# buggyyang/CDC_compression

Measured on AMD Instinct MI355X. Metric: decoded images/sec at 256x256, 500-step x-param, higher is better.
Workload: dtype f32 (f16x2 split products)

## Files before the change

### cdc_compression_amd/csrc/cdc_internal.h

```cpp
#pragma once
#include <stdio.h>
#include <string.h>
#include <stdlib.h>
#include <hip/hip_runtime.h>
#include <map>
#include <mutex>
#include <utility>
#include <stdint.h>

#include <string>
#include <vector>

#include "conv_args.h"

extern "C" char **environ;

namespace cdc {

typedef void (*conv_kernel_fn)(const ConvArgs);
conv_kernel_fn conv_lookup_a(int MB, int NPW, int lnmode);
conv_kernel_fn conv_lookup_b(int MB, int NPW, int lnmode);
conv_kernel_fn conv_lookup_c(int MB, int NPW, int lnmode);
conv_kernel_fn conv_lookup_split(int MB, int NPW);
conv_kernel_fn conv_lookup_split2(int MB, int NPW, int lnmode, int xu = 1);
conv_kernel_fn conv_lookup_split2h(int MB, int NPW, int lnmode, int xu = 1);
conv_kernel_fn conv_lookup_split2hu(int MB, int NPW);

struct ConvShape {
    int Cin, Cout, KH, KW, stride;
    int C0 = 0;
    int Win = 0;
    int nz = 1, pad_x[4] = {0, 0, 0, 0};
    bool allow_split = false;
    int arith = 0;
    bool per_image_w = false;
    int Ho, Wo;
    int B;
    bool need_all_cout;
    int lnmode;
    int max_ksplit = 1;
};
bool conv_make_plan(const ConvShape &s, ConvPlan *plan);
hipError_t conv_launch(ConvArgs a, const ConvPlan &plan, int B, int nz, hipStream_t st);

struct PfShape {
    int Cin, Cout, C0 = 0, KH, KW, nz = 1, Ho, Wo, B;
    bool need_all_cout = false;
    int stride = 1;
    int uf = 0;
    int cop = 0;
    int tz = 1;
};
struct PfPlan {
    int MB, NPW, WM, WP, ring, tiles_x, tiles_y, groups; size_t lds_bytes; int lin = 0;
    int x16 = 0;
    int pf3_epv = 0, pf3_G = 0, pf3_iters = 0;
};
bool pf_make_plan(const PfShape &s, PfPlan *plan);
hipError_t pf_launch(PfArgs a, const PfPlan &plan, int B, int nz, hipStream_t st);
bool pf3_make_plan(const PfArgs &a, int B, int nz, PfPlan *plan);
hipError_t pf3_launch(PfArgs a, const PfPlan &plan, int B, hipStream_t st);
int device_cus();
struct WsPlan { int W, NPB, stride, waves, tiles, groups; size_t lds_bytes; };
struct WsArgs;
bool ws_make_plan(int Cin, int C0, int Cout, int H, int W, int B, int stride, WsPlan *plan);
hipError_t ws_launch(WsArgs a, const WsPlan &plan, hipStream_t st);
struct Ws1Plan { int NPB, waves, tiles, groups; size_t lds_bytes; };
struct Ws1Args;
bool ws1_make_plan(int Cin, int C0, int Cout, int HW, int B, bool per_image_w, Ws1Plan *plan);
hipError_t ws1_launch(Ws1Args a, const Ws1Plan &plan, hipStream_t st);
bool pw_make_plan(const PfShape &s, PfPlan *plan);
hipError_t pw_launch(PfArgs a, const PfPlan &plan, int B, hipStream_t st);
hipError_t pf_pack_launch(const float *src, long long src_bs, void *dst, long long dst_bs, int C, int H, int W, int B,
                          hipStream_t st);
hipError_t c4_pack_launch(const float *src, long long src_bs, float *dst, int C, long long HW, int B, hipStream_t st);
hipError_t pf_unpack_launch(const void *src, long long src_bs, float *dst, long long dst_bs, int C, int H, int W, int B, hipStream_t st);

inline const char *dev_env(const char *name) {
    static const bool on = [] {
        const char *e = ::getenv("CDC_DEV");
        if (e && atoi(e) != 0) return true;
        static const char *const user_level[] = {"CDC_DEV=", "CDC_ARITH=", "CDC_NO_RANGE_GUARD=", "CDC_GRAPH=", "CDC_DEBUG_PLAN=", "CDC_PROF_OPS=",
                                                 "CDC_BENCH_", "CDC_TEST_OBS=", "CDC_SYNC_EACH_OP=", "CDC_HIP_LIB=", "CDC_NO_COMBINE_FUSE="};
        for (char **v = environ; v && *v; ++v) {
            if (strncmp(*v, "CDC_", 4)) continue;
            bool user = false;
            for (const char *u : user_level) user = user || !strncmp(*v, u, strlen(u));
            if (!user) {
                fprintf(stderr, "cdc_hip: %.*s is set but ignored: development switches need CDC_DEV=1\n", (int)strcspn(*v, "="), *v);
                break;
            }
        }
        return false;
    }();
    return on ? ::getenv(name) : nullptr;
}

inline hipError_t ensure_dynamic_lds(const void *fn, size_t bytes) {
    if (bytes <= 64 * 1024) return hipSuccess;
    static std::mutex mu;
    static std::map<std::pair<int, const void *>, size_t> done;
    int dev = 0;
    (void)hipGetDevice(&dev);
    std::lock_guard<std::mutex> lk(mu);
    size_t &have = done[{dev, fn}];
    if (have >= bytes) return hipSuccess;
    hipError_t e = hipFuncSetAttribute(fn, hipFuncAttributeMaxDynamicSharedMemorySize, (int)bytes);
    if (e == hipSuccess) have = bytes;
    return e;
}

__host__ __device__ inline int ceil_div(int a, int b) { return (a + b - 1) / b; }
__host__ __device__ inline int round_up(int a, int b) { return ceil_div(a, b) * b; }

struct LnArgs {
    const float *in;
    float *out;
    int C, HW;
    const float *g, *b;
    float eps;
    int relu;
    const float *shift;
    int shift_bs;
    const float *resid;
    float *stat_mean, *stat_rstd;
    int nparts;
    long long part_stride;
    int *fault;
    int img_major;
};
hipError_t ln_launch(const LnArgs &a, int B, hipStream_t st);

struct TembLayer {
    const float *w, *bias;
    int cout;
    int out_off;
};
struct TembArgs {
// ... 151 lines not shown
```

### cdc_compression_amd/csrc/cdc_planner.hip

```cpp
#include "cdc_state.h"

namespace cdcapi {

constexpr int kKsTarget = 1024;

struct Builder {
    cdc_handle *h;
    int B;
    std::vector<void *> *pool;
    int rc = CDC_OK;
    int planB = 0;
    int pb() const { return planB > 0 ? planB : B; }
    std::vector<Op> *cur = nullptr;

    void emit(Op op) {
        op.id = (int)h->op_ms.size();
        h->op_ms.push_back(0); h->op_n.push_back(0); h->op_flops.push_back(op.flops);
        const bool hoisted = cur == &h->pre_ops;
        char buf[160];
        std::visit([&](const auto &payload) { op_label(payload, buf, sizeof buf, hoisted); }, op.p);
        if (hoisted && !strstr(buf, " HOIST") && strlen(buf) + 7 < sizeof buf) strcat(buf, " HOIST");
        h->op_label.push_back(buf);
        (cur ? cur : &h->ops)->push_back(op);
    }
// ... 249 lines not shown
        if (t0->H != H || t0->W != W || (t1 && (t1->H != H || t1->W != W))) return false;
        if (s1 ? (t0->C != C0 || t0->C + t1->C != w.Cin) : t0->C != w.Cin) return false;
        PfPlan plan;
        if (!pf_make_plan(ps, &plan)) return false;
        const int Ho = ps.Ho, Wo = ps.Wo;
        PfConvOp op;
        op.plan = plan; op.nz = w.nz;
        PfArgs &a = op.a;
        memset(&a, 0, sizeof a);
        a.src0 = t0->p; a.src0_bs = t0->bs();
        if (t1) { a.src1 = t1->p; a.src1_bs = t1->bs(); }
        a.C0 = s1 ? C0 : w.Cin; a.Cin = w.Cin; a.H = H; a.W = W;
        a.w = w.wsh; a.w_zs = w.wsp_zs / 8;
        a.KH = w.KH; a.KW = w.KW; a.nz = w.nz; a.stride = w.stride; a.tz = ps.tz;
        a.nchunk = w.Cin / 16; a.COP = w.COP; a.Cout = w.Cout;
        a.acc_scale = w.wscale_inv;
        out_geometry(a, w, Ho, Wo);
        a.out = out; a.out_bs = out_bs;
        if (o.emit_pf && bind_out_pf(a, w, out, out_bs, Ho, Wo) && o.no_f32) a.out = nullptr;
        epilogue(a, w, o);
        if (o.resid1) {
            if (!o.resid || o.resid_c0 <= 0 || o.resid_c0 >= w.Cout || (o.resid_c0 % 64) || (o.resid_c0 % (plan.MB * 32))) return false;
            a.resid1 = o.resid1; a.resid1_bs = o.resid1_bs; a.resid_c0 = o.resid_c0;
        }
        if (PfTwin *tr = o.resid ? twin(o.resid) : nullptr)
            if (tr->only) {
                if (!tr->valid || tr->C != w.Cout || tr->H != Ho || tr->W != Wo || w.transposed || w.stride != 1 ||
                    o.resid_bs != (long long)w.Cout * Ho * Wo || o.resid_cs != (long long)Ho * Wo) {
                    if (!ensure_f32(o.resid, o.resid_bs)) {
                        if (!rc) rc = fail(h, CDC_ERR_UNSUPPORTED, "planes-only residual of a shape the plane-operand kernels do not read");
                        return true;
                    }
                } else {
                    a.resid = nullptr;
                    a.resid_pf = tr->p; a.rpf_bs = tr->bs(); a.rpf_ps = tr->ps(); a.rpf_ys = Wo + 2; a.rpf_zoff = (Wo + 2) + 1;
                }
            }
        if (planB == 0) pf3_make_plan(a, B, w.nz, &op.plan);
        if (debug_plan())
            fprintf(stderr, "[plan] conv %dx%d %d->%d out %dx%d on conv_pf%s_kernel (epv %d, %d workgroups x %d tiles per group)\n", w.KH, w.KW, w.Cin, w.Cout,
                    Ho, Wo, op.plan.pf3_epv ? "3" : "", op.plan.pf3_epv, op.plan.pf3_G, op.plan.pf3_iters);
        const double px = (double)B * Ho * Wo * w.nz;
        return finish(prof, op, 2.0 * px * w.Cout * w.Cin * w.KH * w.KW, 4.0 * ((double)B * w.Cin * H * W + px * w.Cout), a.out == nullptr);
    }

    bool try_pf_uf(const ConvW &w, const float *s0, long long bs0, int H, int W, float *out, long long out_bs, const ConvOpts &o,
                   bool need_all, int prof) {
        PfShape ps;
        if (!pf_on() || o.uf_c != 3 || o.uf_pad != 3 || !pf_uf_form(w, H, W, need_all, &ps)) return false;
        if (o.pre_mean || o.w_bs || o.wsp_bs || o.max_ksplit > 1 || o.resid || o.res3_w || o.stat_mean) return false;
        PfPlan plan;
        if (!pf_make_plan(ps, &plan)) return false;
        PfConvOp op;
        op.plan = plan; op.nz = 1;
        PfArgs &a = op.a;
        memset(&a, 0, sizeof a);
        a.x0 = s0; a.x0_bs = bs0;
        a.C0 = a.Cin = 32; a.H = H; a.W = W;
        a.w = w.wsh; a.w_zs = w.wsp_zs / 8;
        a.KH = 7; a.KW = 1; a.nz = 1;
        a.nchunk = 2; a.COP = w.COP; a.Cout = w.Cout;
        a.acc_scale = w.wscale_inv;
        out_geometry(a, w, H, W);
        a.out = out; a.out_bs = out_bs;
        if (o.emit_pf && bind_out_pf(a, w, out, out_bs, H, W) && o.no_f32) a.out = nullptr;
        const float *c4 = o.pre_add && cur != &h->pre_ops ? pre_add_c4(o.pre_add, w.Cout, H, W, out_bs) : nullptr;
        epilogue(a, w, o);
        if (c4) { a.pre_add = c4; a.pre_c4 = 1; }
        const double px = (double)B * H * W;
        return finish(prof, op, 2.0 * px * w.Cout * w.Cin * 7, 4.0 * ((double)B * 3 * H * W + px * w.Cout), a.out == nullptr);
    }

    bool try_pw(const ConvW &w, const float *s0, int C0, long long bs0, const float *s1, long long bs1, int H, int W,
                float *out, long long out_bs, const ConvOpts &o, bool need_all, int prof) {
        PfShape ps;
        if (h->arith != 1 || dev_env("CDC_NO_PW") || !pw_form(w, s1 ? C0 : 0, H, W, &ps)) return false;
        if (need_all || o.ln_g || o.stat_mean || o.res3_w || o.pf_only) return false;
        if (o.pre_mean && o.pre_mode != 2) return false;
        if (o.w_bs && !o.wsp_bs) return false;
        PfPlan plan;
        if (!pw_make_plan(ps, &plan)) return false;
        if (plan.lin && (o.shift || o.wsp_bs || (long long)w.Cout * H * W != out_bs)) return false;
        if (debug_plan())
            fprintf(stderr, "[plan] conv1x1 PW Cin=%4d Cout=%4d out=%3dx%-3d %s%s| MB=%d NPW=%d WM=%d WP=%d groups=%d R=%d wgs=%d lds=%zu\n", w.Cin, w.Cout,
                    H, W, o.pre_mean ? "pre2 " : "", o.wsp_bs ? "per-image " : "", plan.MB, plan.NPW, plan.WM, plan.WP, plan.groups, plan.ring,
                    plan.tiles_x * plan.tiles_y * B * plan.groups, plan.lds_bytes);
        PwConvOp op;
        op.plan = plan;
        PfArgs &a = op.a;
        memset(&a, 0, sizeof a);
        a.x0 = s0; a.x0_bs = bs0; a.x1 = s1; a.x1_bs = bs1;
        a.C0 = s1 ? C0 : w.Cin; a.Cin = w.Cin; a.H = H; a.W = W;
        a.pre_mean = o.pre_mean; a.pre_rstd = o.pre_mean ? o.pre_rstd : nullptr;
        a.w = w.wsh; a.w_bs = o.wsp_bs / 8;
        a.KH = 1; a.KW = 1; a.nz = 1;
        a.nchunk = w.Cin / 16; a.COP = w.COP; a.Cout = w.Cout;
        a.acc_scale = w.wscale_inv;
        out_geometry(a, w, H, W);
        a.out = out; a.out_bs = out_bs;
        if (o.emit_pf && !plan.lin && (w.Cout % 32) == 0 && bind_out_pf(a, w, out, out_bs, H, W) && o.no_f32) a.out = nullptr;
        epilogue(a, w, o);
        const double px = (double)B * H * W;
        return finish(prof, op, 2.0 * px * w.Cout * w.Cin, 4.0 * ((double)B * w.Cin * H * W + px * w.Cout), a.out == nullptr);
    }

    bool ws_would_plan(const ConvW &w, int C0, bool two_src, int H, int W, WsPlan *plan) {
        if (h->arith != 1 || !w.wsh || planB > 0 || w.KH != 3 || w.KW != 3 || (w.stride != 1 && w.stride != 2) || w.transposed || w.nz != 1) return false;
        if (w.py() != 1 || w.px() != 1) return false;
        if (w.COP != w.Cout || w.Cin_pad != w.Cin) return false;
        if (w.stride == 2 && ((H & 1) || (W & 1) || two_src)) return false;
        return ws_make_plan(w.Cin, two_src ? C0 : w.Cin, w.Cout, H / w.stride, W / w.stride, pb(), w.stride, plan);
    }
    bool try_ws(const ConvW &w, const float *s0, int C0, long long bs0, const float *s1, long long bs1, int H, int W, float *raw,
                long long raw_bs, int prof, const float *pre_add = nullptr) {
        WsConvOp op;
        if (rc || !ws_would_plan(w, C0, s1 != nullptr, H, W, &op.plan)) return false;
        if (!ensure_f32(s0, bs0) || (s1 && !ensure_f32(s1, bs1))) return false;
        const int Ho = H / w.stride, Wo = W / w.stride;
        if (raw_bs != (long long)w.Cout * Ho * Wo) return false;
        WsArgs &a = op.a;
        memset(&a, 0, sizeof a);
        a.x0 = s0; a.x0_bs = bs0; a.x1 = s1; a.x1_bs = bs1;
        a.C0 = s1 ? C0 : w.Cin; a.Cin = w.Cin; a.H = Ho; a.B = B;
        a.w = w.wsh; a.nchunk = w.Cin / 16; a.COP = w.COP; a.Cout = w.Cout; a.acc_scale = w.wscale_inv;
        a.bias = pre_add ? nullptr : w.bias;
        a.pre_add = pre_add;
        a.out = raw; a.out_bs = raw_bs;
        a.fault = fault_flag();
        if (debug_plan())
            fprintf(stderr, "[plan] conv 3x3 s%d %d->%d out %dx%d on conv_ws_kernel: %d tiles of %d pixels x %d groups, %d waves, %zu bytes of LDS\n", w.stride, w.Cin, w.Cout, Ho, Wo,
                    op.plan.tiles, op.plan.NPB * 32, op.plan.groups, op.plan.waves, op.plan.lds_bytes);
        const double px = (double)B * Ho * Wo;
        return finish(prof, op, 2.0 * px * w.Cout * w.Cin * 9, 4.0 * ((double)B * H * W * w.Cin + px * w.Cout), false);
    }

    bool try_ws1(const ConvW &w, const float *s0, int C0, long long bs0, const float *s1, long long bs1, int H, int W, float *out, long long out_bs,
                 const ConvOpts &o, bool need_all, int prof) {
        PfShape ps;
        if (rc || h->arith != 1 || planB > 0 || !pw_form(w, 0, H, W, &ps)) return false;
        if (need_all || o.ln_g || o.stat_mean || o.res3_w || o.pf_only || (o.pre_add && o.resid) || o.relu || o.resid1 || o.uf_c) return false;
        if (o.pre_mean && o.pre_mode != 2) return false;
        if (o.w_bs && !o.wsp_bs) return false;
        if (w.COP != w.Cout || w.Cin_pad != w.Cin || out_bs != (long long)w.Cout * H * W) return false;
        if (o.resid && (o.resid_cs != (long long)H * W)) return false;
        const long long blocks = (long long)pb() * (H * W / 32);
        const long long max_blocks = dev_env("CDC_WS1_MAX_BLOCKS") ? atoll(dev_env("CDC_WS1_MAX_BLOCKS")) : 128;
        const int max_groups_wide = dev_env("CDC_WS1_MAX_GROUPS") ? atoi(dev_env("CDC_WS1_MAX_GROUPS")) : 0;
        const bool wide_ok = blocks <= max_blocks || (max_groups_wide > 0 && blocks <= 256 && w.Cout / 32 <= max_groups_wide);
        if (!wide_ok && !(o.wsp_bs && W < 32)) return false;
        Ws1ConvOp op;
        op.H = H;
        if (!ws1_make_plan(w.Cin, s1 ? C0 : w.Cin, w.Cout, H * W, pb(), o.wsp_bs != 0, &op.plan)) return false;
        if (!ensure_f32(s0, bs0) || (s1 && !ensure_f32(s1, bs1)) || (o.resid && !ensure_f32(o.resid, o.resid_bs))) return false;
        Ws1Args &a = op.a;
        memset(&a, 0, sizeof a);
        a.x0 = s0; a.x0_bs = bs0; a.x1 = s1; a.x1_bs = bs1;
        a.C0 = s1 ? C0 : w.Cin; a.Cin = w.Cin; a.HW = H * W; a.B = B;
        a.pre_mean = o.pre_mean; a.pre_rstd = o.pre_mean ? o.pre_rstd : nullptr;
        a.w = w.wsh; a.w_bs = o.wsp_bs / 8;
        a.nchunk = w.Cin / 16; a.COP = w.COP; a.Cout = w.Cout; a.acc_scale = w.wscale_inv;
        a.bias = o.no_bias ? nullptr : w.bias;
        a.shift = o.shift; a.shift_bs = shift_stride(o);
        a.resid = o.resid; a.resid_bs = o.resid_bs;
        if (o.pre_add) { a.resid = o.pre_add; a.resid_bs = out_bs; a.resid_is_pre = 1; }
        a.out = out; a.out_bs = out_bs;
        a.fault = fault_flag();
        if (debug_plan())
            fprintf(stderr, "[plan] conv 1x1 %d->%d out %dx%d on conv_ws1_kernel: %d tiles of %d pixels x %d groups, %d waves%s%s\n", w.Cin, w.Cout, H, W,
                    op.plan.tiles, op.plan.NPB * 32, op.plan.groups, op.plan.waves, o.pre_mean ? ", folded PreNorm" : "", o.wsp_bs ? ", per-image weights" : "");
// ... 1072 lines not shown
```

### cdc_compression_amd/csrc/conv_args.h

```cpp
#pragma once
#include <stdint.h>

namespace cdc {

constexpr int kWaveSize = 64;
constexpr int kXS = 20;

struct ConvArgs {
    const float *src0, *src1;
    long long src0_bs, src1_bs;
    int uf_c, uf_pad;
    unsigned uf_magic;
    int C0, Cin;
    int H, W;
    const float *ln_mean, *ln_rstd;
    const float *ln_g, *ln_b;
    const float *wp;
    long long w_bs, w_zs;
    const unsigned short *wsp;
    long long wsp_zs;
    long long wsp_bs;
    float acc_scale;
    int tg;
    int ipw, B;
// ... 3 lines not shown
    float *out;
    long long out_bs, out_cs;
    int out_ys, out_xs, out_zoff[4];
    int Ho, Wo;
    int lognbw;
    int tiles_x, tiles_y;
    int PH, PW;
    int xvec, xshift[4];
    unsigned magic_hw, magic_w;
    const float *bias;
    const float *pre_add;
    const float *ep_g, *ep_b;
    float eps;
    int relu;
    float relu_slope;
    const float *shift;
    int shift_bs;
    const float *resid;
    long long resid_bs, resid_cs;
    const float *res3_w, *res3_x;
    long long res3_bs;
    float *stat_mean, *stat_rstd;
    int ksplit, nzz;
    int xcd_remap;
    int zfold;
    long long out_ks;
    void *out_pf;
    long long pf_bs, pf_ps;
    int pf_ys, pf_xs, pf_zoff[4];
    int pf_only;
    int *fault;
#ifdef CDC_TIMELINE
    unsigned long long *tl;
#endif
};

struct PfArgs {
    const void *src0, *src1;
    long long src0_bs, src1_bs;
    int C0, Cin;
    int H, W;
    const void *w;
    long long w_zs;
    int KH, KW, nz;
    int stride;
    int tz;
    int pad_y[4], pad_x[4];
    int nchunk, COP, Cout;
    float acc_scale;
    int ring;
    int n_iter;
    float *out;
    long long out_bs, out_cs;
    int out_ys, out_xs, out_zoff[4];
    void *out_pf;
    long long pf_bs, pf_ps;
    int pf_ys, pf_xs, pf_zoff[4];
    int Ho, Wo;
    int lognbw, tiles_x, tiles_y, B;
    int xcd_remap;
    const float *bias, *pre_add, *ep_g, *ep_b;
    int pre_c4;
    float eps;
    int relu;
    float relu_slope;
    const float *shift;
    int shift_bs;
    const float *resid;
    long long resid_bs, resid_cs;
    const float *resid1;
    long long resid1_bs;
    int resid_c0;
    const void *resid_pf;
    long long rpf_bs, rpf_ps;
    int rpf_ys, rpf_zoff;
    float *stat_mean, *stat_rstd;
    const float *res3_w, *res3_x;
    long long res3_bs;
    const float *x0, *x1;
    long long x0_bs, x1_bs;
    const float *pre_mean, *pre_rstd;
    long long w_bs;
    int lin;
    int dbg;
    int *fault;
#ifdef CDC_TIMELINE
    unsigned long long *tl;
#endif
};

constexpr int kPfXS = 12;

struct ConvPlan {
    int MB, NPW, WN;
    int groups;
    int KC, nchunk;
    int lognbw, tiles_x, tiles_y, PH, PW;
    int xvec, xshift[4];
    size_t lds_bytes;
    int lnmode;
    int tg;
    int ipw;
    int ksplit = 1;
    int xu = 1;
    int arith = 0;
    int split;
};

}
```

### cdc_compression_amd/csrc/conv_inst_w.hip

```cpp
#include <algorithm>
#include <map>
#include <string>
#include <vector>
#include <stdlib.h>

#include "cdc_internal.h"
#include "conv_pw_kernel.h"

namespace cdc {

typedef void (*pw_kernel_fn)(const PfArgs);
static pw_kernel_fn pw_lookup(int MB, int NPW, int WM, int WP, bool x16 = false) {
    if (x16) {
        if (MB == 2 && NPW == 2 && WM == 1 && WP == 4) return conv_pw_kernel<2, 2, 1, 4, true>;
        if (MB == 2 && NPW == 2 && WM == 2 && WP == 2) return conv_pw_kernel<2, 2, 2, 2, true>;
        if (MB == 2 && NPW == 2 && WM == 4 && WP == 2) return conv_pw_kernel<2, 2, 4, 2, true>;
        if (MB == 3 && NPW == 1 && WM == 2 && WP == 4) return conv_pw_kernel<3, 1, 2, 4, true>;
        return nullptr;
    }
    if (MB == 2 && NPW == 2 && WM == 1 && WP == 4) return conv_pw_kernel<2, 2, 1, 4>;
    if (MB == 2 && NPW == 2 && WM == 2 && WP == 2) return conv_pw_kernel<2, 2, 2, 2>;
    if (MB == 2 && NPW == 2 && WM == 4 && WP == 2) return conv_pw_kernel<2, 2, 4, 2>;
    if (MB == 3 && NPW == 1 && WM == 2 && WP == 4) return conv_pw_kernel<3, 1, 2, 4>;
    return nullptr;
}
struct PwCand { int MB, NPW, WM, WP; };
static const PwCand kPwCands[] = {
    {2, 2, 4, 2},
    {3, 1, 2, 4},
    {2, 2, 2, 2},
    {2, 2, 1, 4},
};

bool pw_make_plan(const PfShape &s, PfPlan *p) {
    if (s.KH != 1 || s.KW != 1 || s.nz != 1) return false;
    if (s.Cout % 32 || s.Cin % 16 || (s.C0 % 16) || s.Cin < 32) return false;
    const bool lin = s.Wo < 32;
    if (lin && ((s.Ho * s.Wo) % 32)) return false;
    const double min_waves = dev_env("CDC_PW_MIN_WAVES") ? atof(dev_env("CDC_PW_MIN_WAVES")) : 512.0;
    const bool x16 = (lin || ((s.Wo & 3) == 0 && s.Wo >= 4)) && !dev_env("CDC_NO_PW_X16");
    double best = -1;
    for (const PwCand &c : kPwCands) {
        const int COPT = c.WM * c.MB * 32, NW = c.WM * c.WP;
        if (s.Cout % COPT) continue;
        if (s.need_all_cout && COPT != s.Cout) continue;
        const int ring = pw_ring(c.MB, c.NPW, c.WM, c.WP, x16);
        if (ring < 5 || s.Cin / 16 < 2) continue;
        const int TH = c.WP * c.NPW;
        const int groups = s.Cout / COPT;
        const long long nb = (long long)s.B * (s.Ho * s.Wo / 32);
        const double wgs = lin ? (double)((nb + TH - 1) / TH) * groups
                               : (double)((s.Wo + 31) / 32) * ((s.Ho + TH - 1) / TH) * s.B * groups;
        if (wgs * NW < min_waves) continue;
        const double fill = std::min(1.0, wgs * NW / 2048.0);
        const double score = fill / (1.0 + 0.25 * (groups - 1)) * (c.MB * c.NPW >= 4 ? 1.0 : 0.8);
        if (score > best) {
            best = score;
            p->MB = c.MB; p->NPW = c.NPW; p->WM = c.WM; p->WP = c.WP;
            p->ring = ring;
            p->lin = lin ? 1 : 0;
            p->tiles_x = lin ? (int)((nb + TH - 1) / TH) : (s.Wo + 31) / 32;
            p->tiles_y = lin ? 1 : (s.Ho + TH - 1) / TH;
            p->groups = groups;
            p->lds_bytes = (size_t)ring * pf_rows(c.MB, c.NPW) * COPT * 16 + pw_x_bytes(c.NPW, c.WM, c.WP, x16);
            p->x16 = x16 ? 1 : 0;
        }
    }
    return best >= 0;
}

hipError_t pw_launch(PfArgs a, const PfPlan &p, int B, hipStream_t st) {
    pw_kernel_fn fn = pw_lookup(p.MB, p.NPW, p.WM, p.WP, p.x16 != 0);
    if (!fn) return hipErrorInvalidValue;
    a.lognbw = 5;
    a.tiles_x = p.tiles_x; a.tiles_y = p.tiles_y; a.B = B; a.ring = p.ring;
    if (hipError_t e = ensure_dynamic_lds((const void *)fn, p.lds_bytes); e != hipSuccess) return e;
    a.lin = p.lin;
    if (const char *e = dev_env("CDC_PW_DBG")) a.dbg = atoi(e); else
    a.dbg = dev_env("CDC_PW_COUNTED_WAIT") ? 1024 : 0;
    dim3 grid((unsigned)(p.lin ? p.tiles_x : p.tiles_x * p.tiles_y * B), (unsigned)p.groups, 1);
    a.xcd_remap = (grid.x % 8 == 0 && grid.x >= 64) ? 1 : 0;
#ifdef CDC_TIMELINE
    static unsigned long long *tl_dev = nullptr;
    static std::map<std::string, int> seen;
    const size_t tl_wgs = (size_t)grid.x * grid.y;
    char key[96];
    snprintf(key, sizeof key, "pw 1x1 %d->%d out %dx%d", a.Cin, a.Cout, a.Ho, a.Wo);
    a.tl = nullptr;
    if (tl_wgs <= (1u << 18) && seen[key]++ < 2) {
        if (!tl_dev) hipMalloc(&tl_dev, sizeof(unsigned long long) * 16 * (1u << 18));
        hipMemsetAsync(tl_dev, 0, sizeof(unsigned long long) * 16 * tl_wgs, st);
        a.tl = tl_dev;
    }
#endif
    hipLaunchKernelGGL(fn, grid, dim3(64 * p.WM * p.WP), p.lds_bytes, st, a);
#ifdef CDC_TIMELINE
    if (a.tl) {
        hipStreamSynchronize(st);
        std::vector<unsigned long long> h(16 * tl_wgs);
        hipMemcpy(h.data(), tl_dev, h.size() * 8, hipMemcpyDeviceToHost);
        double cat[7] = {0}, life = 0;
        for (size_t w = 0; w < tl_wgs; ++w) {
            const unsigned long long *r = &h[w * 16];
            for (int c = 0; c < 7; ++c) cat[c] += (double)r[c];
            life += (double)(r[8] - r[7]);
        }
        static const char *names[7] = {"setup", "prologue issue", "prologue wait", "main loop", "epilogue parameters", "-", "epilogue blocks"};
        fprintf(stderr, "[pf timeline] conv %s: %zu workgroups x %d threads, lds %zu; mean workgroup life %.0f; per workgroup (wave 0):", key, tl_wgs, 64 * p.WM * p.WP, p.lds_bytes,
                life / tl_wgs);
        for (int c = 0; c < 7; ++c) fprintf(stderr, "  %s %.0f", names[c], cat[c] / tl_wgs);
        fprintf(stderr, "\n");
    }
#endif
    return hipGetLastError();
}

}
```

### cdc_compression_amd/csrc/conv_pw_kernel.h

```cpp
#pragma once
#include "conv_pf_kernel.h"

namespace cdc {

constexpr int kPwPD = 2;
constexpr int kPwX16N = 2 * 256 + 32;
__host__ __device__ constexpr size_t pw_x_bytes(int NPW, int WM, int WP, bool X16 = false) {
    return (size_t)WM * WP * kPwPD * NPW * (X16 ? kPwX16N * 4 : 8 * 256);
}
__host__ __device__ constexpr int pw_ring(int MB, int NPW, int WM, int WP, bool X16 = false) {
    const size_t budget = (WM * WP == 8 ? 150 * 1024 : 78 * 1024) - pw_x_bytes(NPW, WM, WP, X16);
    const size_t wst = (size_t)pf_rows(MB, NPW) * WM * MB * 32 * 16;
    const int r = (int)(budget / wst);
    return r > 6 ? 6 : r;
}

__device__ __forceinline__ void dma4(unsigned voff, const void *sbase, unsigned lds_byte) {
    asm volatile("s_mov_b32 m0, %2\n\ts_nop 0\n\tglobal_load_lds_dword %0, %1" ::"v"(voff), "s"(sbase), "s"(lds_byte)
                 : "memory");
}

template <int MB, int NPW, int WM, int WP, bool X16 = false>
__global__ void __launch_bounds__(64 * WM * WP, WM * WP == 8 ? 1 : 2) conv_pw_kernel(const PfArgs P) {
    constexpr int NW = WM * WP, NT = 64 * NW, COPT = WM * MB * 32;
    static_assert(COPT % 64 == 0, "a weight DMA instruction (64 units) must stay inside one (plane, k-half) row");
    constexpr bool ACC2 = pf_acc2(MB, NPW);
    constexpr int NPL = ACC2 ? 2 : 3, ROWS = 2 * NPL;
    constexpr int WI = ROWS * COPT / 64;
    constexpr int NWW = (WI + NW - 1) / NW;
    constexpr int WST = ROWS * COPT;
    constexpr int R = pw_ring(MB, NPW, WM, WP, X16);
    static_assert(R >= 5, "no room for the weight ring");
    constexpr int TH = WP * NPW;
    constexpr int PD = kPwPD;
    extern __shared__ __attribute__((aligned(16))) uint4 smem_u[];
#ifdef CDC_TIMELINE
    unsigned long long tl_acc[7] = {0, 0, 0, 0, 0, 0, 0}, tl_last = __builtin_readcyclecounter();
    const unsigned long long tl_start = tl_last;
#endif
    const int tid = threadIdx.x, lane = tid & 63;
    const int wave = __builtin_amdgcn_readfirstlane(tid >> 6);
    const int wm = wave / WP, wp = wave % WP;
    const int cog = blockIdx.y;
    unsigned bid0 = blockIdx.x;
    if (P.xcd_remap) bid0 = (bid0 & 7) * (gridDim.x >> 3) + (bid0 >> 3);
    int bid = (int)bid0;
    const int tile = bid;
    const int tx = bid % P.tiles_x;
    bid /= P.tiles_x;
    const int ty = bid % P.tiles_y;
    const int b = P.lin ? 0 : bid / P.tiles_y;
    const int oy0 = ty * TH, ox0 = tx * 32;
    const int S = P.nchunk;
    const unsigned lds0 = __builtin_amdgcn_readfirstlane((unsigned)(size_t)(const __attribute__((address_space(3))) uint4 *)smem_u);

    const char *wsrc = reinterpret_cast<const char *>(P.w) + ((size_t)b * P.w_bs + (size_t)cog * COPT) * 16;
    unsigned wvo[NWW], wdo[NWW];
#pragma unroll
    for (int k = 0; k < NWW; ++k) {
        const int jj = min(wave + k * NW, WI - 1);
        const int row = jj / (COPT / 64), seg = jj - row * (COPT / 64);
        wvo[k] = (unsigned)(row * P.COP + seg * 64 + lane) * 16u;
        wdo[k] = __builtin_amdgcn_readfirstlane((unsigned)jj * 1024u);
    }
    const long long w_dc = (long long)6 * P.COP * 16;
    const char *wptr = wsrc;
    int sw = 0;
    auto issue_w = [&]() {
        const unsigned dst = lds0 + (unsigned)(sw * WST) * 16u;
#pragma unroll
        for (int k = 0; k < NWW; ++k) dma16(wvo[k], wptr, dst + wdo[k]);
        wptr += w_dc;
        if (++sw == R) sw = 0;
    };

    const int half = lane >> 5, j = lane & 31;
    const int HW = P.H * P.W;
    unsigned xvo[NPW];
    float mu[NPW];
    bool valid[NPW];
    unsigned pixo[NPW];
    int bimg[NPW];
    const int bpi = HW >> 5;
#pragma unroll
    for (int n = 0; n < NPW; ++n) {
        if (P.lin) {
            const int gb = tile * TH + wp * NPW + n, nb = P.B * bpi;
            valid[n] = gb < nb;
            const int gc = min(gb, nb - 1);
            bimg[n] = __builtin_amdgcn_readfirstlane(gc / bpi);
            pixo[n] = (unsigned)((gc - bimg[n] * bpi) * 32 + j);
        } else {
            const int oy = oy0 + wp * NPW + n, ox = ox0 + j;
            valid[n] = oy < P.Ho && ox < P.Wo;
            bimg[n] = b;
            pixo[n] = (unsigned)(min(oy, P.Ho - 1) * P.W + min(ox, P.Wo - 1));
        }
        xvo[n] = ((unsigned)(8 * half) * (unsigned)HW + pixo[n]) * 4u;
        if constexpr (X16) {
            const int r = lane >> 3, q = lane & 7;
            unsigned p4;
            if (P.lin) p4 = pixo[n] - (unsigned)j + 4u * q;
            else {
                const int oy = oy0 + wp * NPW + n;
                p4 = (unsigned)(min(oy, P.Ho - 1) * P.W + min(ox0 + 4 * q, P.Wo - 4));
            }
            xvo[n] = ((unsigned)r * (unsigned)HW + p4) * 4u;
        }
        mu[n] = P.pre_mean ? P.pre_mean[(size_t)bimg[n] * HW + pixo[n]] : 0.f;
    }
    const int c0_chunks = P.C0 >> 4;
    constexpr int L = (X16 ? 2 : 8) * NPW;
    constexpr int XST = X16 ? NPW * kPwX16N : NPW * 8 * 64;
    float *xw = reinterpret_cast<float *>(smem_u + R * WST) + wave * (PD * XST);
    const unsigned xw_lds = lds0 + (unsigned)(R * WST) * 16u + (unsigned)(wave * (PD * XST)) * 4u;
    auto issue_x = [&](int c, int slot) {
        const unsigned dst = xw_lds + (unsigned)(slot * XST) * 4u;
#pragma unroll
        for (int n = 0; n < NPW; ++n) {
            const float *src = c < c0_chunks ? P.x0 + (size_t)bimg[n] * P.x0_bs + (size_t)c * 16 * HW
                                             : P.x1 + (size_t)bimg[n] * P.x1_bs + (size_t)(c - c0_chunks) * 16 * HW;
            const char *base = reinterpret_cast<const char *>(uniform_ptr(src));
            if constexpr (X16) {
#pragma unroll
                for (int hh = 0; hh < 2; ++hh) dma16(xvo[n], base + (size_t)(8 * hh) * HW * 4, dst + (unsigned)(n * kPwX16N + hh * (256 + 32)) * 4u);
            } else {
#pragma unroll
            for (int i = 0; i < 8; ++i) dma4(xvo[n], base + (size_t)i * HW * 4, dst + (unsigned)((n * 8 + i) * 64) * 4u);
            }
        }
    };

    f32x16 acc[MB][NPW], acc2[ACC2 ? MB : 1][ACC2 ? NPW : 1];
#pragma unroll
    for (int m = 0; m < MB; ++m)
#pragma unroll
        for (int n = 0; n < NPW; ++n)
#pragma unroll
            for (int r = 0; r < 16; ++r) {
                acc[m][n][r] = 0.f;
                if constexpr (ACC2) acc2[m][n][r] = 0.f;
            }
    const uint4 *a_base = smem_u + half * COPT + wm * MB * 32 + j;
    typedef f16x8 OpsA[NPL][MB];
    typedef f16x8 OpsB[2][NPW];
    auto fetch_a = [&](const uint4 *wa, OpsA &A) {
#pragma unroll
        for (int pl = 0; pl < NPL; ++pl)
#pragma unroll
            for (int m = 0; m < MB; ++m) A[pl][m] = __builtin_bit_cast(f16x8, wa[(pl * 2) * COPT + m * 32]);
    };
    auto split_b = [&](int slot, OpsB &Bv) {
        const float *src = xw + slot * XST + (X16 ? half * (256 + 32) + j : lane);
#pragma unroll
        for (int n = 0; n < NPW; ++n)
#pragma unroll
            for (int i = 0; i < 8; ++i) {
                _Float16 hq, lq;
                split2h((X16 ? src[n * kPwX16N + i * 32] : src[(n * 8 + i) * 64]) - mu[n], hq, lq);
                Bv[0][n][i] = hq; Bv[1][n][i] = lq;
            }
    };
    auto mma = [&](const OpsA &A, const OpsB &Bv) {
        if constexpr (ACC2) {
#pragma unroll
            for (int m = 0; m < MB; ++m)
#pragma unroll
                for (int n = 0; n < NPW; ++n) acc[m][n] = __builtin_amdgcn_mfma_f32_32x32x16_f16(A[1][m], Bv[0][n], acc[m][n], 0, 0, 0);
#pragma unroll
            for (int m = 0; m < MB; ++m)
#pragma unroll
                for (int n = 0; n < NPW; ++n) acc2[m][n] = __builtin_amdgcn_mfma_f32_32x32x16_f16(A[0][m], Bv[1][n], acc2[m][n], 0, 0, 0);
#pragma unroll
            for (int m = 0; m < MB; ++m)
#pragma unroll
                for (int n = 0; n < NPW; ++n) acc[m][n] = __builtin_amdgcn_mfma_f32_32x32x16_f16(A[0][m], Bv[0][n], acc[m][n], 0, 0, 0);
        } else {
#pragma unroll
            for (int term = 0; term < 3; ++term) {
                constexpr int PA[3] = {1, 2, 0};
                constexpr int PB[3] = {0, 1, 0};
#pragma unroll
                for (int m = 0; m < MB; ++m)
#pragma unroll
                    for (int n = 0; n < NPW; ++n)
                        acc[m][n] = __builtin_amdgcn_mfma_f32_32x32x16_f16(A[PA[term] % NPL][m], Bv[PB[term]][n], acc[m][n], 0, 0, 0);
            }
        }
    };

    PFTL(0);
#pragma unroll
    for (int d = 0; d < PD; ++d)
        if (d < S) issue_x(d, d);
    for (int q = 0; q < R - 1 && q < S; ++q) issue_w();
    PFTL(1);
    dma_wait();
    __builtin_amdgcn_s_barrier();
    PFTL(2);
    OpsA A0, A1;
    OpsB B0, B1;
    fetch_a(a_base, A0);
    split_b(0, B0);
    if (PD < S) issue_x(PD, 0);
    int sn = 0;
    auto step = [&](int s, auto slotc, OpsA &Ac, OpsB &Bc, OpsA &An, OpsB &Bn) {
        constexpr int slot = decltype(slotc)::value;
        if (s + 1 < S) {
            if (++sn == R) sn = 0;
            if (s >= PD && s + R - 1 < S && s + 1 + PD < S && (P.dbg & 1024)) {
                if (P.dbg & 2048) vm_wait<(PD - 1) * (L + NWW)>(); else vm_wait<NWW + (PD - 1) * (L + NWW)>();
                if (P.dbg & 4096) __builtin_amdgcn_s_sleep(4);
            } else dma_wait();
            __builtin_amdgcn_s_barrier();
            fetch_a(a_base + sn * WST, An);
            split_b(slot, Bn);
#ifdef CDC_PW_LATE_PROBE
            if (P.dbg & 8192) {
                if (P.dbg & 16384) __builtin_amdgcn_s_sleep(16);
                OpsB Bt;
                split_b(slot, Bt);
                unsigned late = 0;
#pragma unroll
                for (int n = 0; n < NPW; ++n) {
                    bool d = false;
#pragma unroll
                    for (int i = 0; i < 8; ++i) d |= (float)Bn[0][n][i] != (float)Bt[0][n][i] || (float)Bn[1][n][i] != (float)Bt[1][n][i];
                    if (__any(d)) late |= 1u << n;
                }
                if (late && lane == 0)
                    printf("[pw late piece] workgroup (%d,%d) wave %d step %d of %d: pixel-block mask %x differs between the read behind vmcnt(%d) and a second read\n",
                           (int)blockIdx.x, (int)blockIdx.y, wave, s + 1, S, late, NWW + (PD - 1) * (L + NWW));
            }
#endif
            if (s + 1 + PD < S) issue_x(s + 1 + PD, slot);
            if (s + R - 1 < S) issue_w();
        }
        __builtin_amdgcn_s_setprio(2);
        mma(Ac, Bc);
        __builtin_amdgcn_s_setprio(0);
    };
    static_assert(PD == 2 && R >= PD + 3, "two activation stages; W(s+1) must be older than the activation pieces of step s+1");
    using P0 = std::integral_constant<int, 0>;
    using P1 = std::integral_constant<int, 1>;
    {
        int s = 0;
        for (; s + 1 < S; s += 2) {
            step(s, P1{}, A0, B0, A1, B1);
            step(s + 1, P0{}, A1, B1, A0, B0);
        }
        if (s < S) step(s, P1{}, A0, B0, A1, B1);
    }

    __builtin_amdgcn_s_barrier();
    PFTL(3);
    float *ep = reinterpret_cast<float *>(smem_u);
    for (int i = tid; i < COPT; i += NT) {
        const int co = cog * COPT + i;
        const bool ok = co < P.Cout;
        ep[i] = (ok && P.bias) ? P.bias[co] : 0.f;
        ep[COPT + i] = (ok && P.shift) ? P.shift[(size_t)b * P.shift_bs + co] : 0.f;
    }
    __syncthreads();
    PFTL(4);
    const int cobase = cog * COPT + wm * MB * 32;
    const float *epl = ep + wm * MB * 32 + 4 * half;
    const bool ch_ok = cobase + MB * 32 <= P.Cout;
#pragma unroll
    for (int n = 0; n < NPW; ++n) {
        const int oy = oy0 + wp * NPW + n, ox = ox0 + j;
        const int bn = bimg[n];
        const bool ok = valid[n] && ch_ok;
        const float sc = P.pre_rstd ? P.acc_scale * P.pre_rstd[(size_t)bn * HW + pixo[n]] : P.acc_scale;
        const size_t opix = P.lin ? (size_t)pixo[n] : (size_t)oy * P.out_ys + (size_t)ox * P.out_xs + P.out_zoff[0];
#pragma unroll
        for (int m = 0; m < MB; ++m)
#pragma unroll
            for (int r = 0; r < 16; ++r)
                acc[m][n][r] = (ACC2 ? acc[m][n][r] + acc2[ACC2 ? m : 0][ACC2 ? n : 0][r] * (1.0f / 2048.0f) : acc[m][n][r]) * sc +
                               epl[m * 32 + (r & 3) + 8 * (r >> 2)];
        if (!ok) continue;
        if (P.fault) {
            float s = 0.f;
#pragma unroll
            for (int m = 0; m < MB; ++m)
#pragma unroll
                for (int r = 0; r < 16; ++r) s += fabsf(acc[m][n][r]);
            if (!(s < 3.0e38f)) *P.fault = 1;
        }
        if (P.pre_add) {
// ... 45 lines not shown
```

Baseline: 5.430.

## Share split f16 activation planes across waves in pointwise conv kernel

Adds a shared-split mode to the 1x1 pointwise conv kernel. Each wave DMAs only its slice of the activation chunk, splits it to hi/lo f16 once, and publishes it to a shared LDS plane that all waves in the same pixel column read. Previously every wave split its own copy. This removes redundant global loads and split arithmetic, at the cost of an extra LDS publish plus barrier per step and less LDS for the weight ring. It also folds the Cout group index into the x-dimension grid ordering so that groups sharing the same pixels are scheduled together after the XCD remap.

Result: no change. 5.454 (median of 6 runs) (+0.4%).

```diff
diff --git a/cdc_compression_amd/csrc/cdc_internal.h b/cdc_compression_amd/csrc/cdc_internal.h
--- a/cdc_compression_amd/csrc/cdc_internal.h
+++ b/cdc_compression_amd/csrc/cdc_internal.h
@@ -54,6 +54,8 @@
 struct PfPlan {
     int MB, NPW, WM, WP, ring, tiles_x, tiles_y, groups; size_t lds_bytes; int lin = 0;
     int x16 = 0;
+    int sh = 0;
+    int gord = 0;
     int pf3_epv = 0, pf3_G = 0, pf3_iters = 0;
 };
 bool pf_make_plan(const PfShape &s, PfPlan *plan);
diff --git a/cdc_compression_amd/csrc/cdc_planner.hip b/cdc_compression_amd/csrc/cdc_planner.hip
--- a/cdc_compression_amd/csrc/cdc_planner.hip
+++ b/cdc_compression_amd/csrc/cdc_planner.hip
@@ -355,9 +355,9 @@
         if (!pw_make_plan(ps, &plan)) return false;
         if (plan.lin && (o.shift || o.wsp_bs || (long long)w.Cout * H * W != out_bs)) return false;
         if (debug_plan())
-            fprintf(stderr, "[plan] conv1x1 PW Cin=%4d Cout=%4d out=%3dx%-3d %s%s| MB=%d NPW=%d WM=%d WP=%d groups=%d R=%d wgs=%d lds=%zu\n", w.Cin, w.Cout,
-                    H, W, o.pre_mean ? "pre2 " : "", o.wsp_bs ? "per-image " : "", plan.MB, plan.NPW, plan.WM, plan.WP, plan.groups, plan.ring,
-                    plan.tiles_x * plan.tiles_y * B * plan.groups, plan.lds_bytes);
+            fprintf(stderr, "[plan] conv1x1 PW Cin=%4d Cout=%4d out=%3dx%-3d %s%s%s| MB=%d NPW=%d WM=%d WP=%d groups=%d R=%d wgs=%d lds=%zu %s%s\n", w.Cin, w.Cout,
+                    H, W, o.pre_mean ? "pre2 " : "", o.wsp_bs ? "per-image " : "", s1 ? "two-source " : "", plan.MB, plan.NPW, plan.WM, plan.WP, plan.groups, plan.ring,
+                    plan.tiles_x * plan.tiles_y * B * plan.groups, plan.lds_bytes, plan.sh ? "shared-split" : "per-wave", plan.lin ? " lin" : "");
         PwConvOp op;
         op.plan = plan;
         PfArgs &a = op.a;
diff --git a/cdc_compression_amd/csrc/conv_args.h b/cdc_compression_amd/csrc/conv_args.h
--- a/cdc_compression_amd/csrc/conv_args.h
+++ b/cdc_compression_amd/csrc/conv_args.h
@@ -109,6 +109,7 @@
     const float *pre_mean, *pre_rstd;
     long long w_bs;
     int lin;
+    int pw_groups;
     int dbg;
     int *fault;
 #ifdef CDC_TIMELINE
diff --git a/cdc_compression_amd/csrc/conv_inst_w.hip b/cdc_compression_amd/csrc/conv_inst_w.hip
--- a/cdc_compression_amd/csrc/conv_inst_w.hip
+++ b/cdc_compression_amd/csrc/conv_inst_w.hip
@@ -10,7 +10,14 @@
 namespace cdc {
 
 typedef void (*pw_kernel_fn)(const PfArgs);
-static pw_kernel_fn pw_lookup(int MB, int NPW, int WM, int WP, bool x16 = false) {
+static pw_kernel_fn pw_lookup(int MB, int NPW, int WM, int WP, bool x16 = false, bool sh = false) {
+    if (sh) {
+        if (!x16) return nullptr;
+        if (MB == 2 && NPW == 2 && WM == 2 && WP == 2) return conv_pw_kernel<2, 2, 2, 2, true, true>;
+        if (MB == 2 && NPW == 2 && WM == 4 && WP == 2) return conv_pw_kernel<2, 2, 4, 2, true, true>;
+        if (MB == 3 && NPW == 1 && WM == 2 && WP == 4) return conv_pw_kernel<3, 1, 2, 4, true, true>;
+        return nullptr;
+    }
     if (x16) {
         if (MB == 2 && NPW == 2 && WM == 1 && WP == 4) return conv_pw_kernel<2, 2, 1, 4, true>;
         if (MB == 2 && NPW == 2 && WM == 2 && WP == 2) return conv_pw_kernel<2, 2, 2, 2, true>;
@@ -39,12 +46,14 @@
     if (lin && ((s.Ho * s.Wo) % 32)) return false;
     const double min_waves = dev_env("CDC_PW_MIN_WAVES") ? atof(dev_env("CDC_PW_MIN_WAVES")) : 512.0;
     const bool x16 = (lin || ((s.Wo & 3) == 0 && s.Wo >= 4)) && !dev_env("CDC_NO_PW_X16");
+    const bool sh_on = x16 && !dev_env("CDC_NO_PW_SHARED") && !dev_env("CDC_PW_DBG") && !dev_env("CDC_PW_COUNTED_WAIT");
     double best = -1;
     for (const PwCand &c : kPwCands) {
         const int COPT = c.WM * c.MB * 32, NW = c.WM * c.WP;
         if (s.Cout % COPT) continue;
         if (s.need_all_cout && COPT != s.Cout) continue;
-        const int ring = pw_ring(c.MB, c.NPW, c.WM, c.WP, x16);
+        const bool sh = sh_on && pw_sh_ok(c.NPW, c.WM) && (c.WM >= 4 || dev_env("CDC_PW_SHARED_WM2"));
+        const int ring = pw_ring(c.MB, c.NPW, c.WM, c.WP, x16, sh);
         if (ring < 5 || s.Cin / 16 < 2) continue;
         const int TH = c.WP * c.NPW;
         const int groups = s.Cout / COPT;
@@ -62,15 +71,16 @@
             p->tiles_x = lin ? (int)((nb + TH - 1) / TH) : (s.Wo + 31) / 32;
             p->tiles_y = lin ? 1 : (s.Ho + TH - 1) / TH;
             p->groups = groups;
-            p->lds_bytes = (size_t)ring * pf_rows(c.MB, c.NPW) * COPT * 16 + pw_x_bytes(c.NPW, c.WM, c.WP, x16);
+            p->lds_bytes = (size_t)ring * pf_rows(c.MB, c.NPW) * COPT * 16 + pw_x_bytes(c.NPW, c.WM, c.WP, x16, sh);
             p->x16 = x16 ? 1 : 0;
+            p->sh = sh ? 1 : 0;
         }
     }
     return best >= 0;
 }
 
 hipError_t pw_launch(PfArgs a, const PfPlan &p, int B, hipStream_t st) {
-    pw_kernel_fn fn = pw_lookup(p.MB, p.NPW, p.WM, p.WP, p.x16 != 0);
+    pw_kernel_fn fn = pw_lookup(p.MB, p.NPW, p.WM, p.WP, p.x16 != 0, p.sh != 0);
     if (!fn) return hipErrorInvalidValue;
     a.lognbw = 5;
     a.tiles_x = p.tiles_x; a.tiles_y = p.tiles_y; a.B = B; a.ring = p.ring;
@@ -80,6 +90,11 @@
     a.dbg = dev_env("CDC_PW_COUNTED_WAIT") ? 1024 : 0;
     dim3 grid((unsigned)(p.lin ? p.tiles_x : p.tiles_x * p.tiles_y * B), (unsigned)p.groups, 1);
     a.xcd_remap = (grid.x % 8 == 0 && grid.x >= 64) ? 1 : 0;
+    a.pw_groups = 0;
+    if (p.groups > 1 && p.WM * p.WP == 8 && a.xcd_remap && !dev_env("CDC_NO_PW_GROUP_ORDER")) {
+        a.pw_groups = p.groups;
+        grid = dim3(grid.x * (unsigned)p.groups, 1, 1);
+    }
 #ifdef CDC_TIMELINE
     static unsigned long long *tl_dev = nullptr;
     static std::map<std::string, int> seen;
diff --git a/cdc_compression_amd/csrc/conv_pw_kernel.h b/cdc_compression_amd/csrc/conv_pw_kernel.h
--- a/cdc_compression_amd/csrc/conv_pw_kernel.h
+++ b/cdc_compression_amd/csrc/conv_pw_kernel.h
@@ -5,11 +5,16 @@
 
 constexpr int kPwPD = 2;
 constexpr int kPwX16N = 2 * 256 + 32;
-__host__ __device__ constexpr size_t pw_x_bytes(int NPW, int WM, int WP, bool X16 = false) {
+__host__ __device__ constexpr int pw_sh_pieces(int NPW, int WM) { return 2 * NPW / WM; }
+__host__ __device__ constexpr int pw_sh_raw_floats(int NPW, int WM) { return pw_sh_pieces(NPW, WM) == 2 ? kPwX16N : 256; }
+__host__ __device__ constexpr size_t pw_sh_plane_bytes(int NPW, int WP) { return (size_t)2 * WP * NPW * 2 * 64 * 16; }
+__host__ __device__ constexpr bool pw_sh_ok(int NPW, int WM) { return WM > 1 && (2 * NPW) % WM == 0 && 2 * NPW / WM <= 2; }
+__host__ __device__ constexpr size_t pw_x_bytes(int NPW, int WM, int WP, bool X16 = false, bool SH = false) {
+    if (SH) return pw_sh_plane_bytes(NPW, WP) + (size_t)WM * WP * kPwPD * pw_sh_raw_floats(NPW, WM) * 4;
     return (size_t)WM * WP * kPwPD * NPW * (X16 ? kPwX16N * 4 : 8 * 256);
 }
-__host__ __device__ constexpr int pw_ring(int MB, int NPW, int WM, int WP, bool X16 = false) {
-    const size_t budget = (WM * WP == 8 ? 150 * 1024 : 78 * 1024) - pw_x_bytes(NPW, WM, WP, X16);
+__host__ __device__ constexpr int pw_ring(int MB, int NPW, int WM, int WP, bool X16 = false, bool SH = false) {
+    const size_t budget = (WM * WP == 8 ? 150 * 1024 : 78 * 1024) - pw_x_bytes(NPW, WM, WP, X16, SH);
     const size_t wst = (size_t)pf_rows(MB, NPW) * WM * MB * 32 * 16;
     const int r = (int)(budget / wst);
     return r > 6 ? 6 : r;
@@ -20,8 +25,9 @@
                  : "memory");
 }
 
-template <int MB, int NPW, int WM, int WP, bool X16 = false>
+template <int MB, int NPW, int WM, int WP, bool X16 = false, bool SH = false>
 __global__ void __launch_bounds__(64 * WM * WP, WM * WP == 8 ? 1 : 2) conv_pw_kernel(const PfArgs P) {
+    static_assert(!SH || (X16 && pw_sh_ok(NPW, WM)), "shared split: 16-byte pieces, one or two of them per wave and step");
     constexpr int NW = WM * WP, NT = 64 * NW, COPT = WM * MB * 32;
     static_assert(COPT % 64 == 0, "a weight DMA instruction (64 units) must stay inside one (plane, k-half) row");
     constexpr bool ACC2 = pf_acc2(MB, NPW);
@@ -29,7 +35,7 @@
     constexpr int WI = ROWS * COPT / 64;
     constexpr int NWW = (WI + NW - 1) / NW;
     constexpr int WST = ROWS * COPT;
-    constexpr int R = pw_ring(MB, NPW, WM, WP, X16);
+    constexpr int R = pw_ring(MB, NPW, WM, WP, X16, SH);
     static_assert(R >= 5, "no room for the weight ring");
     constexpr int TH = WP * NPW;
     constexpr int PD = kPwPD;
@@ -41,9 +47,13 @@
     const int tid = threadIdx.x, lane = tid & 63;
     const int wave = __builtin_amdgcn_readfirstlane(tid >> 6);
     const int wm = wave / WP, wp = wave % WP;
-    const int cog = blockIdx.y;
+    int cog = blockIdx.y;
     unsigned bid0 = blockIdx.x;
     if (P.xcd_remap) bid0 = (bid0 & 7) * (gridDim.x >> 3) + (bid0 >> 3);
+    if (P.pw_groups) {
+        cog = (int)(bid0 % (unsigned)P.pw_groups);
+        bid0 /= (unsigned)P.pw_groups;
+    }
     int bid = (int)bid0;
     const int tile = bid;
     const int tx = bid % P.tiles_x;
@@ -107,13 +117,86 @@
             }
             xvo[n] = ((unsigned)r * (unsigned)HW + p4) * 4u;
         }
-        mu[n] = P.pre_mean ? P.pre_mean[(size_t)bimg[n] * HW + pixo[n]] : 0.f;
+        mu[n] = (!SH && P.pre_mean) ? P.pre_mean[(size_t)bimg[n] * HW + pixo[n]] : 0.f;
+    }
+    constexpr int PPW = SH ? pw_sh_pieces(NPW, WM) : 0;
+    const int cn = (wm * PPW) >> 1, chh = (wm * PPW) & 1;
+    unsigned cxvo = 0;
+    int cimg = 0;
+    float cmu = 0.f;
+    if constexpr (SH) {
+        const int q = lane & 7;
+        unsigned pix, p4;
+        if (P.lin) {
+            const int gc = min(tile * TH + wp * NPW + cn, P.B * bpi - 1);
+            cimg = __builtin_amdgcn_readfirstlane(gc / bpi);
+            pix = (unsigned)((gc - cimg * bpi) * 32 + j);
+            p4 = pix - (unsigned)j + 4u * q;
+        } else {
+            const int oy = min(oy0 + wp * NPW + cn, P.Ho - 1);
+            cimg = b;
+            pix = (unsigned)(oy * P.W + min(ox0 + j, P.Wo - 1));
+            p4 = (unsigned)(oy * P.W + min(ox0 + 4 * q, P.Wo - 4));
+        }
+        cxvo = ((unsigned)(lane >> 3) * (unsigned)HW + p4) * 4u;
+        cmu = P.pre_mean ? P.pre_mean[(size_t)cimg * HW + pix] : 0.f;
     }
     const int c0_chunks = P.C0 >> 4;
     constexpr int L = (X16 ? 2 : 8) * NPW;
     constexpr int XST = X16 ? NPW * kPwX16N : NPW * 8 * 64;
-    float *xw = reinterpret_cast<float *>(smem_u + R * WST) + wave * (PD * XST);
-    const unsigned xw_lds = lds0 + (unsigned)(R * WST) * 16u + (unsigned)(wave * (PD * XST)) * 4u;
+    constexpr int XSS = SH ? pw_sh_raw_floats(NPW, WM) : 0;
+    constexpr int XPU = SH ? (int)(pw_sh_plane_bytes(NPW, WP) / 16) : 0;
+    uint4 *xpl = smem_u + R * WST;
+    float *xw = reinterpret_cast<float *>(smem_u + R * WST + XPU) + wave * (PD * (SH ? XSS : XST));
+    const unsigned xw_lds = lds0 + (unsigned)(R * WST + XPU) * 16u + (unsigned)(wave * (PD * (SH ? XSS : XST))) * 4u;
+    auto issue_xs = [&](int c, int slot) {
+        const float *src = c < c0_chunks ? P.x0 + (size_t)cimg * P.x0_bs + (size_t)c * 16 * HW
+                                         : P.x1 + (size_t)cimg * P.x1_bs + (size_t)(c - c0_chunks) * 16 * HW;
+        const char *base = reinterpret_cast<const char *>(uniform_ptr(src));
+        const unsigned dst = xw_lds + (unsigned)(slot * XSS) * 4u;
+        if constexpr (PPW == 2) {
+#pragma unroll
+            for (int hh = 0; hh < 2; ++hh) dma16(cxvo, base + (size_t)(8 * hh) * HW * 4, dst + (unsigned)(hh * (256 + 32)) * 4u);
+        } else dma16(cxvo, base + (size_t)(8 * chh) * HW * 4, dst);
+    };
+    auto publish = [&](int slot, int buf) {
+        const float *src = xw + slot * XSS;
+        uint4 *dst = xpl + ((buf * WP + wp) * NPW + cn) * 128;
+        if constexpr (PPW == 2) {
+            f16x8 hv, lv;
+#pragma unroll
+            for (int i = 0; i < 8; ++i) {
+                _Float16 hq, lq;
+                split2h(src[half * (256 + 32) + i * 32 + j] - cmu, hq, lq);
+                hv[i] = hq; lv[i] = lq;
+            }
+            dst[lane] = __builtin_bit_cast(uint4, hv);
+            dst[64 + lane] = __builtin_bit_cast(uint4, lv);
+        } else {
+            f16x4 hv, lv;
+#pragma unroll
+            for (int i = 0; i < 4; ++i) {
+                _Float16 hq, lq;
+                split2h(src[(4 * half + i) * 32 + j] - cmu, hq, lq);
+                hv[i] = hq; lv[i] = lq;
+            }
+            reinterpret_cast<uint2 *>(dst + chh * 32 + j)[half] = __builtin_bit_cast(uint2, hv);
+            reinterpret_cast<uint2 *>(dst + 64 + chh * 32 + j)[half] = __builtin_bit_cast(uint2, lv);
+        }
+    };
+    auto read_b = [&](int buf, auto &Bv) {
+        const uint4 *src = xpl + (buf * WP + wp) * NPW * 128 + lane;
+#pragma unroll
+        for (int n = 0; n < NPW; ++n) {
+            Bv[0][n] = __builtin_bit_cast(f16x8, src[n * 128]);
+            Bv[1][n] = __builtin_bit_cast(f16x8, src[n * 128 + 64]);
+        }
+    };
+    auto publish_barrier = [&]() {
+        asm volatile("s_waitcnt lgkmcnt(0)" ::: "memory");
+        __builtin_amdgcn_s_barrier();
+        asm volatile("" ::: "memory");
+    };
     auto issue_x = [&](int c, int slot) {
         const unsigned dst = xw_lds + (unsigned)(slot * XST) * 4u;
 #pragma unroll
@@ -192,20 +275,44 @@
     PFTL(0);
 #pragma unroll
     for (int d = 0; d < PD; ++d)
-        if (d < S) issue_x(d, d);
+        if (d < S) { if constexpr (SH) issue_xs(d, d); else issue_x(d, d); }
     for (int q = 0; q < R - 1 && q < S; ++q) issue_w();
     PFTL(1);
     dma_wait();
+    OpsA A0, A1;
+    OpsB B0, B1;
+    if constexpr (SH) {
+#pragma unroll
+        for (int d = 0; d < PD; ++d) {
+            if (d < S) publish(d, d);
+            if (d + PD < S) issue_xs(d + PD, d);
+        }
+        publish_barrier();
+        PFTL(2);
+        fetch_a(a_base, A0);
+        read_b(0, B0);
+    } else {
     __builtin_amdgcn_s_barrier();
     PFTL(2);
-    OpsA A0, A1;
-    OpsB B0, B1;
     fetch_a(a_base, A0);
     split_b(0, B0);
     if (PD < S) issue_x(PD, 0);
+    }
     int sn = 0;
     auto step = [&](int s, auto slotc, OpsA &Ac, OpsB &Bc, OpsA &An, OpsB &Bn) {
         constexpr int slot = decltype(slotc)::value;
+        if constexpr (SH) {
+            if (s + 1 < S) {
+                if (++sn == R) sn = 0;
+                dma_wait();
+                publish_barrier();
+                fetch_a(a_base + sn * WST, An);
+                read_b(slot, Bn);
+                if (s + 2 < S) publish(1 - slot, 1 - slot);
+                if (s + 2 + PD < S) issue_xs(s + 2 + PD, 1 - slot);
+                if (s + R - 1 < S) issue_w();
+            }
+        } else
         if (s + 1 < S) {
             if (++sn == R) sn = 0;
             if (s >= PD && s + R - 1 < S && s + 1 + PD < S && (P.dbg & 1024)) {
```
